# ibm-granite/dolomite-engine

Hardware: NVIDIA H100
Metric: tokens_per_sec (higher is better)
Workload: dtype bf16

## Files before the change

dolomite_engine_b200/csrc/gemm.cu:

```cuda
#include <string.h>

#include "common.cuh"
#include "wgmma.cuh"
#include "../../include/dolomite_b200.h"

using namespace dolo;

namespace {

constexpr int BM = 128;
constexpr int BN = 128;
constexpr int BK = 64;
constexpr int A_STAGE_BYTES = BM * BK * 2;
constexpr int GEMM_THREADS = 384;

constexpr int EPI_SLAB_BYTES = 64 * 128;
constexpr int EPI_BYTES = 2  * 2  * EPI_SLAB_BYTES;
constexpr int EPI_BIAS_BYTES = 2  * 256 * 2;

template <int TN>
struct Ring {
    static_assert(TN == 128 || TN == 256, "tile width 128 or 256");
    static constexpr int STAGES = TN == 256 ? 4 : 6;
    static constexpr int B_BYTES = TN * BK * 2;
// ... 429 lines not shown
            const uint32_t sb = smem_u32(smem_b + stage * B_STAGE_BYTES);
#pragma unroll
            for (int k = 0; k < 4; ++k) {
                const uint64_t adesc = A_MN ? gmma_desc(sa + cw * (BK * 128) + k * 2048, BK * 128, 1024, 1)
                                            : gmma_desc(sa + cw * (64 * 128) + k * 32, 16, 1024, 1);
                const uint64_t bdesc = B_MN ? gmma_desc(sb + k * 2048, BK * 128, 1024, 1)
                                            : gmma_desc(sb + k * 32, 16, 1024, 1);
                Op::template mma<TN>(acc, adesc, bdesc, ((!Op::SPLIT && kb != ti.kb0) || k != 0) ? 1u : 0u);
            }
            wgmma_commit();
            if (kb == min(ti.kb0 + 2, ti.kb1 - 1) && has_c && epi.leader) epi.load_c_prefetch(&maps.c[ti.q], chunk_cols, col0, row0, dgrp);
            if constexpr (Op::SPLIT) {
                wgmma_wait<0>();
                reg_fence<TN / 2>(acc);
                if (lane == 0) mbar_arrive(&empty_bar[stage]);
                if (kb == ti.kb0) {
#pragma unroll
                    for (int i = 0; i < TN / 2; ++i) tot[i] = acc[i];
                } else {
#pragma unroll
                    for (int i = 0; i < TN / 2; ++i) tot[i] += acc[i];
                }
            } else {
                wgmma_wait<1>();
                if (prev_stage >= 0 && lane == 0) mbar_arrive(&empty_bar[prev_stage]);
                prev_stage = stage;
            }
            if (++stage == STAGES) { stage = 0; phase ^= 1; }
        }
        if constexpr (!Op::SPLIT) {
            wgmma_wait<0>();
            reg_fence<TN / 2>(acc);
            if (prev_stage >= 0 && lane == 0) mbar_arrive(&empty_bar[prev_stage]);
        }
        const float(&res)[TN / 2] = Op::SPLIT ? tot : acc;
        float s = 1.f;
        if constexpr (Op::SCALED) s = __ldg(p.a_scale_inv[ti.q]) * __ldg(p.b_scale_inv[ti.q]);
        if (has_bias && wt < TN / 2) epi.bias[wt] = bias_v;
        epi.begin_tile();

        if (p.d_is_f32)
            epi.store<TN, true, Op::SCALED>(res, &maps.d[ti.q], &maps.c[ti.q], col0, row0, dgrp, s, pr.alpha, pr.beta,
                                            has_bias, has_c, Op::GROUPED && p.grouped == 3);
        else
            epi.store<TN, false, Op::SCALED>(res, &maps.d[ti.q], &maps.c[ti.q], col0, row0, dgrp, s, pr.alpha, pr.beta,
                                             has_bias, has_c, false);
    }
    if (epi.leader) tma_store_wait_all<0>();
}

template <bool A_MN, bool B_MN, int TN>
__global__ void __launch_bounds__(GEMM_THREADS, 1)
    gemm_bf16_kernel(const __grid_constant__ GemmMaps maps, const __grid_constant__ GemmParams p) {
    gemm_body<Bf16Ops<A_MN, B_MN>, TN>(maps, p);
}

template <int FA, int FB, bool SPLIT>
__global__ void __launch_bounds__(GEMM_THREADS, 1)
    gemm_fp8_kernel(const __grid_constant__ GemmMaps maps, const __grid_constant__ GemmParams p) {
    gemm_body<Fp8Ops<FA, FB, SPLIT>, 128>(maps, p);
}

int gemm_workers() {
    const int sms = dolo_num_sms() - dolo_option_gemm_sm_margin();
    return sms < 1 ? 1 : sms;
}

template <int TN, void (*KERNEL)(GemmMaps, GemmParams)>
int launch_gemm(const GemmMaps& maps, const GemmParams& p, cudaStream_t st) {
    constexpr int smem_bytes = Ring<TN>::SMEM_BYTES;
    static bool attr_set = false;
    if (!attr_set) {
        DOLO_CUDA_OK(cudaFuncSetAttribute(KERNEL, cudaFuncAttributeMaxDynamicSharedMemorySize, smem_bytes));
        attr_set = true;
    }
    const int sms = gemm_workers();
    const int grid = p.num_tiles < sms ? p.num_tiles : sms;
    KERNEL<<<grid, GEMM_THREADS, smem_bytes, st>>>(maps, p);
    DOLO_LAUNCH_OK("gemm");
    return DOLO_OK;
}

int choose_tile_n(int n, const int64_t* M, const int64_t* N) {
    const int forced = dolo_option_gemm_tile_n();
    if (forced != 0) return forced;
    const int64_t w = gemm_workers();
    int64_t t128 = 0, t256 = 0;
    for (int q = 0; q < n; ++q) {
        const int64_t mb = (M[q] + BM - 1) / BM;
        t128 += mb * ((N[q] + 127) / 128);
        t256 += mb * ((N[q] + 255) / 256);
    }
    const double c128 = double((t128 + w - 1) / w);
    const double c256 = double((t256 + w - 1) / w) * TILE256_COST;
    return c256 < c128 ? 256 : 128;
}

}

struct GroupArgs {
    int mode = 0;
    const int* a_row_index = nullptr;
    int64_t a_rows = 0;
    const int* m_tile_group = nullptr;
    int64_t b_group_rows = 0;
    const int* group_k_offsets = nullptr;
    int num_groups = 1;
    int64_t d_group_stride = 0;
    int64_t b_total_outer = 0;
    int64_t bias_group_stride = 0;
};

struct GemmProblemArgs {
    const void* A; int64_t lda;
    const void* B; int64_t ldb;
    void* D; int64_t ldd;
    const void* C; int64_t ldc;
    const void* bias;
    float alpha, beta;
    int64_t M, N, K;
    const float* a_scale_inv = nullptr;
    const float* b_scale_inv = nullptr;
};

static int setup_problem(GemmMaps& maps, GemmParams& p, int q, const GemmProblemArgs& g, int ab, int a_mn_major,
                         int b_mn_major, int d_is_f32, const GroupArgs& ga, int tile_n) {
    const int64_t M = g.M, N = g.N, K = g.K;
    if (ab == 1) {
        DOLO_REQUIRE(M > 0 && N > 0 && K > 0, "gemm_fp8: empty problem (M=%lld N=%lld K=%lld)", (long long)M,
                     (long long)N, (long long)K);
        DOLO_REQUIRE(K % 16 == 0 && N % 16 == 0, "gemm_fp8: K=%lld and N=%lld must be multiples of 16", (long long)K,
                     (long long)N);
        DOLO_REQUIRE(g.lda % 16 == 0 && g.ldb % 16 == 0 && g.lda >= K && g.ldb >= K,
                     "gemm_fp8: lda / ldb must be >= K and multiples of 16 (16-byte aligned fp8 rows)");
        DOLO_REQUIRE(g.a_scale_inv != nullptr && g.b_scale_inv != nullptr, "gemm_fp8: missing scale_inv pointer");
        p.a_scale_inv[q] = g.a_scale_inv;
        p.b_scale_inv[q] = g.b_scale_inv;
    }
    DOLO_REQUIRE(K > 0, "gemm: K must be > 0");
    DOLO_REQUIRE(g.lda * ab % 16 == 0 && g.ldb * ab % 16 == 0 && g.ldd % (d_is_f32 ? 4 : 8) == 0,
                 "gemm: leading dimensions must keep 16-byte alignment");
    {
        const int64_t per = d_is_f32 ? 4 : 8;
        DOLO_REQUIRE(g.ldd >= (N + per - 1) / per * per,
                     "gemm: ldd=%lld must cover N=%lld rounded up to 16 bytes (the TMA store writes that segment)",
                     (long long)g.ldd, (long long)N);
    }
    DOLO_REQUIRE(g.C == nullptr || g.ldc % (d_is_f32 ? 4 : 8) == 0, "gemm: ldc alignment");
    DOLO_REQUIRE((reinterpret_cast<uintptr_t>(g.bias) & 3) == 0, "gemm: bias must be 4-byte aligned");
    DOLO_REQUIRE(M < (1ll << 31) && N < (1ll << 31) && K < (1ll << 31), "gemm: dimension too large");
// ... 30 lines not shown
        rc = dolo_make_tmap(&maps.b[q], g.B, ab, 3, dims3, strides3, box3, DOLO_SW_128);
    } else {
        dims[0] = uint64_t(N); dims[1] = uint64_t(K); strides[1] = uint64_t(g.ldb) * 2;
        box[0] = 64; box[1] = BK;
        rc = dolo_make_tmap(&maps.b[q], g.B, ab, 2, dims, strides, box, DOLO_SW_128);
    }
    if (rc) return rc;
    {
        const uint64_t eb = d_is_f32 ? 4 : 2;
        const int64_t groups = ga.mode == 2 ? ga.num_groups : 1;
        const int64_t group_stride = ga.mode == 2 ? ga.d_group_stride : M * g.ldd;
        uint64_t ddims[3] = {uint64_t(N), uint64_t(M), uint64_t(groups)};
        uint64_t dstrides[3] = {eb, uint64_t(g.ldd) * eb, uint64_t(group_stride) * eb};
        const uint32_t dbox[3] = {uint32_t(128 / eb), 64, 1};
        rc = dolo_make_tmap(&maps.d[q], g.D, int(eb), 3, ddims, dstrides, dbox, DOLO_SW_128);
        if (rc) return rc;
        if (g.C != nullptr) {
            dstrides[1] = uint64_t(g.ldc) * eb;
            if (ga.mode != 2) dstrides[2] = uint64_t(M * g.ldc) * eb;
            rc = dolo_make_tmap(&maps.c[q], g.C, int(eb), 3, ddims, dstrides, dbox, DOLO_SW_128);
            if (rc) return rc;
        }
    }
    Problem& pr = p.pr[q];
    pr.D = g.D;
    pr.C = g.C;
    pr.bias = static_cast<const __nv_bfloat16*>(g.bias);
    pr.ldd = g.ldd;
    pr.ldc = g.ldc;
    pr.M = int(M);
    pr.N = int(N);
    pr.alpha = g.alpha;
    pr.beta = g.C ? g.beta : 0.f;
    pr.hint_a = pr.hint_b = TMA_HINT_NORMAL;
    if (ab == 2 && dolo_option_gemm_l2_hints() && ga.mode == 0 && K >= 4096 && (M + N) * K * 2 > (24ll << 20)) {
        const bool a_smaller = M <= N;
        pr.hint_a = a_smaller ? TMA_HINT_EVICT_LAST : TMA_HINT_EVICT_FIRST;
        pr.hint_b = a_smaller ? TMA_HINT_EVICT_FIRST : TMA_HINT_EVICT_LAST;
    }
    pr.num_m = int((M + BM - 1) / BM);
    pr.num_n = int((N + tile_n - 1) / tile_n);
    pr.num_kb = int((K * ab + 127) / 128);
    {
        const int64_t panel_bytes = int64_t(BM) * K * ab;
        int64_t gm = (12ll << 20) / (panel_bytes > 0 ? panel_bytes : 1);
        if (gm < 4) gm = 4;
        if (gm > 64) gm = 64;
        pr.group_m = int(gm);
    }
    return DOLO_OK;
}

template <int TN>
static int dispatch_layout(int a_mn_major, int b_mn_major, const GemmMaps& maps, const GemmParams& p, cudaStream_t st) {
    if (!a_mn_major && !b_mn_major) return launch_gemm<TN, gemm_bf16_kernel<false, false, TN>>(maps, p, st);
    if (!a_mn_major && b_mn_major) return launch_gemm<TN, gemm_bf16_kernel<false, true, TN>>(maps, p, st);
    if (a_mn_major && !b_mn_major) return launch_gemm<TN, gemm_bf16_kernel<true, false, TN>>(maps, p, st);
    return launch_gemm<TN, gemm_bf16_kernel<true, true, TN>>(maps, p, st);
}

static int dispatch(int tile_n, int a_mn_major, int b_mn_major, const GemmMaps& maps, const GemmParams& p, cudaStream_t st) {
    return tile_n == 256 ? dispatch_layout<256>(a_mn_major, b_mn_major, maps, p, st)
                         : dispatch_layout<128>(a_mn_major, b_mn_major, maps, p, st);
}

template <int FA, int FB>
static int dispatch_fp8_split(int split, const GemmMaps& maps, const GemmParams& p, cudaStream_t st) {
    return split ? launch_gemm<BN, gemm_fp8_kernel<FA, FB, true>>(maps, p, st)
                 : launch_gemm<BN, gemm_fp8_kernel<FA, FB, false>>(maps, p, st);
}

static int dispatch_fp8(int a_fmt, int b_fmt, int split, const GemmMaps& maps, const GemmParams& p, cudaStream_t st) {
    if (a_fmt == 0 && b_fmt == 0) return dispatch_fp8_split<0, 0>(split, maps, p, st);
    if (a_fmt == 0 && b_fmt == 1) return dispatch_fp8_split<0, 1>(split, maps, p, st);
    if (a_fmt == 1 && b_fmt == 0) return dispatch_fp8_split<1, 0>(split, maps, p, st);
    return dispatch_fp8_split<1, 1>(split, maps, p, st);
}

static int gemm_impl(const void* A, int64_t lda, int a_mn_major, const void* B, int64_t ldb, int b_mn_major, void* D,
                     int64_t ldd, int d_is_f32, const void* C, int64_t ldc, float alpha, float beta, const void* bias,
                     int64_t M, int64_t N, int64_t K, int flags, void* stream, const GroupArgs& ga) {
    DOLO_REQUIRE(M >= 0 && N >= 0 && K >= 0, "gemm: negative dimension");
    if (M == 0 || N == 0) return DOLO_OK;
    const bool tma_store = (flags & DOLO_GEMM_FLAG_TMA_STORE) != 0;
    DOLO_REQUIRE(!tma_store || (!d_is_f32 && C == nullptr), "gemm: TMA-store epilogue needs bf16 D and no C");
    const int tile_n = ga.mode == 0 ? choose_tile_n(1, &M, &N) : BN;
    GemmMaps maps;
    GemmParams p;
    memset(&p, 0, sizeof(p));
    GemmProblemArgs g{A, lda, B, ldb, D, ldd, C, ldc, bias, alpha, beta, M, N, K};
    int rc = setup_problem(maps, p, 0, g, 2, a_mn_major, b_mn_major, d_is_f32, ga, tile_n);
    if (rc) return rc;
    p.n_prob = 1;
    p.pr[0].tile_start = 0;
    p.num_tiles = p.pr[0].num_m * p.pr[0].num_n * (ga.mode >= 2 ? ga.num_groups : 1);
    p.d_is_f32 = d_is_f32;
    p.grouped = ga.mode;
    p.m_tile_group = ga.m_tile_group;
    p.a_row_index = ga.a_row_index;
    p.b_group_rows = int(ga.b_group_rows);
    p.group_k_offsets = ga.group_k_offsets;
    p.num_groups = ga.num_groups;
    p.bias_group_stride = ga.bias_group_stride;
    return dispatch(tile_n, a_mn_major, b_mn_major, maps, p, static_cast<cudaStream_t>(stream));
}

extern "C" int dolomite_b200_gemm_bf16_wgrad_multi(int n_problems, const void* const* dY, const int64_t* ld_dy,
                                                   const void* const* X, const int64_t* ld_x, float* const* dW,
                                                   const int64_t* ld_dw, const int64_t* M, const int64_t* N, int64_t K,
                                                   const float* alpha, const int* accumulate, void* stream) {
    DOLO_REQUIRE(n_problems >= 1 && n_problems <= MAXP, "wgrad_multi: between 1 and %d problems per launch", MAXP);
    for (int q = 0; q < n_problems; ++q) DOLO_REQUIRE(M[q] > 0 && N[q] > 0, "wgrad_multi: empty problem %d", q);
    const int tile_n = choose_tile_n(n_problems, M, N);
    GemmMaps maps;
    GemmParams p;
    memset(&p, 0, sizeof(p));
    int tiles = 0;
    for (int q = 0; q < n_problems; ++q) {
        GemmProblemArgs g{dY[q], ld_dy[q], X[q], ld_x[q], dW[q], ld_dw[q], accumulate[q] ? dW[q] : nullptr, ld_dw[q], nullptr,
                          alpha[q], 1.f, M[q], N[q], K};
        int rc = setup_problem(maps, p, q, g, 2, 1, 1, 1, GroupArgs(), tile_n);
        if (rc) return rc;
        p.pr[q].tile_start = tiles;
        tiles += p.pr[q].num_m * p.pr[q].num_n;
    }
    p.n_prob = n_problems;
    p.num_tiles = tiles;
    p.d_is_f32 = 1;
    p.grouped = 0;
    p.num_groups = 1;
    return dispatch(tile_n, 1, 1, maps, p, static_cast<cudaStream_t>(stream));
}

extern "C" int dolomite_b200_gemm_bf16_tile_n(int n_problems, const int64_t* M, const int64_t* N, int* tile_n,
                                              float* cost_256_over_128) {
    DOLO_REQUIRE(n_problems >= 1 && n_problems <= MAXP && M != nullptr && N != nullptr && tile_n != nullptr,
                 "gemm_bf16_tile_n: between 1 and %d problems, non-null M, N and tile_n", MAXP);
    *tile_n = choose_tile_n(n_problems, M, N);
    if (cost_256_over_128 != nullptr) *cost_256_over_128 = float(TILE256_COST);
    return DOLO_OK;
}

extern "C" int dolomite_b200_gemm_bf16(const void* A, int64_t lda, int a_mn_major, const void* B, int64_t ldb,
                                       int b_mn_major, void* D, int64_t ldd, int d_is_f32, const void* C, int64_t ldc,
                                       float alpha, float beta, const void* bias, int64_t M, int64_t N, int64_t K,
                                       int flags, void* stream) {
    if (flags & DOLO_GEMM_FLAG_SPLITK_ACCUMULATE) {
        DOLO_REQUIRE(d_is_f32 && bias == nullptr && (C == nullptr || (C == D && beta == 1.f)),
                     "gemm: split-K accumulate needs fp32 D, no bias and C == D with beta == 1");
        const int64_t tiles = ((M + BM - 1) / BM) * ((N + BN - 1) / BN);
        const int64_t num_kb = (K + BK - 1) / BK;
        const int sms = dolo_num_sms();
        int best_s = 1;
        double best = 1e30;
        for (int s = 1; s <= 16; ++s) {
            if (s > 1 && num_kb / s < 8) break;
            const double waves = double((tiles * s + sms - 1) / sms) / double(s);
            if (waves < best - 1e-9) { best = waves; best_s = s; }
        }
        GroupArgs ga;
        ga.mode = 3;
        ga.num_groups = best_s;
        return gemm_impl(A, lda, a_mn_major, B, ldb, b_mn_major, D, ldd, 1, nullptr, 0, alpha, 0.f, nullptr, M, N, K, 0,
                         stream, ga);
    }
    return gemm_impl(A, lda, a_mn_major, B, ldb, b_mn_major, D, ldd, d_is_f32, C, ldc, alpha, beta, bias, M, N, K, flags,
                     stream, GroupArgs());
}

static int grouped_m_impl(const void* A, int64_t lda, int64_t a_rows, const int32_t* a_row_index, const void* B,
                          int64_t ldb, int b_mn_major, void* D, int64_t ldd, const void* bias, int64_t ld_bias,
                          float alpha, int64_t M_max, int64_t N, int64_t K, const int32_t* m_tile_group, int num_groups,
                          int flags, void* stream) {
    DOLO_REQUIRE(M_max % BM == 0, "grouped gemm: M_max=%lld must be a multiple of %d (padded expert segments)",
                 (long long)M_max, BM);
    DOLO_REQUIRE(!b_mn_major || K % 8 == 0, "grouped gemm: MN-major B needs K %% 8 == 0 (K=%lld)", (long long)K);
    DOLO_REQUIRE(m_tile_group != nullptr && num_groups > 0, "grouped gemm: missing group table");
    if (a_row_index != nullptr) {
        DOLO_REQUIRE(!b_mn_major && a_rows > 0, "grouped gemm (gather): K-major B and a_rows > 0 needed");
        DOLO_REQUIRE((reinterpret_cast<uintptr_t>(a_row_index) & 15) == 0,
                     "grouped gemm (gather): row index must be 16-byte aligned");
    }
    DOLO_REQUIRE(bias == nullptr || (ld_bias >= N && ld_bias % 2 == 0),
                 "grouped gemm: ld_bias=%lld must be even and >= N=%lld", (long long)ld_bias, (long long)N);
    GroupArgs ga;
    ga.mode = 1;
    ga.a_row_index = a_row_index;
    ga.a_rows = a_rows;
    ga.m_tile_group = m_tile_group;
    ga.num_groups = num_groups;
    ga.b_group_rows = N;
    ga.b_total_outer = N * num_groups;
    ga.bias_group_stride = bias != nullptr ? ld_bias : 0;
    return gemm_impl(A, lda, 0, B, ldb, b_mn_major, D, ldd, 0, nullptr, 0, alpha, 0.f, bias, M_max, N, K, flags, stream,
                     ga);
}

extern "C" int dolomite_b200_gemm_bf16_grouped_m(const void* A, int64_t lda, const void* B, int64_t ldb, int b_mn_major,
                                                 void* D, int64_t ldd, float alpha, int64_t M_max, int64_t N, int64_t K,
                                                 const int32_t* m_tile_group, int num_groups, int flags, void* stream) {
    return grouped_m_impl(A, lda, 0, nullptr, B, ldb, b_mn_major, D, ldd, nullptr, 0, alpha, M_max, N, K, m_tile_group,
                          num_groups, flags, stream);
}

extern "C" int dolomite_b200_gemm_bf16_grouped_m_gather(const void* A, int64_t lda, int64_t a_rows,
                                                        const int32_t* a_row_index, const void* B, int64_t ldb, void* D,
                                                        int64_t ldd, float alpha, int64_t M_max, int64_t N, int64_t K,
                                                        const int32_t* m_tile_group, int num_groups, int flags,
                                                        void* stream) {
    DOLO_REQUIRE(a_row_index != nullptr, "grouped gemm (gather): missing row index");
    return grouped_m_impl(A, lda, a_rows, a_row_index, B, ldb, 0, D, ldd, nullptr, 0, alpha, M_max, N, K, m_tile_group,
                          num_groups, flags, stream);
}

extern "C" int dolomite_b200_gemm_bf16_grouped_m_bias(const void* A, int64_t lda, int64_t a_rows,
                                                      const int32_t* a_row_index, const void* B, int64_t ldb,
                                                      int b_mn_major, void* D, int64_t ldd, const void* bias,
                                                      int64_t ld_bias, float alpha, int64_t M_max, int64_t N, int64_t K,
                                                      const int32_t* m_tile_group, int num_groups, int flags,
                                                      void* stream) {
// ... 67 lines not shown
```

dolomite_engine_b200/_lib.py:

```python

from __future__ import annotations

import ctypes
import os
from ctypes import c_char_p, c_float, c_int, c_int64, c_uint32, c_void_p

_HERE = os.path.dirname(os.path.abspath(__file__))
LIB_PATH = os.path.join(_HERE, "lib", "libdolomite_b200.so")


class DolomiteB200Error(RuntimeError):
    pass


_P = c_void_p
_I = c_int
_L = c_int64
_F = c_float
_U = c_uint32

SIGNATURES: dict[str, tuple] = {
    "dolomite_b200_last_error": (c_char_p, []),
    "dolomite_b200_abi_version": (_I, []),
    "dolomite_b200_device_info": (_I, [_P, _P, _P]),
    "dolomite_b200_set_option": (_I, [c_char_p, _I]),
    "dolomite_b200_get_option": (_I, [c_char_p, _P]),
    "dolomite_b200_rmsnorm_fwd": (_I, [_P, _P, _P, _P, _L, _I, _F, _P]),
    "dolomite_b200_rmsnorm_bwd_workspace_bytes": (_L, [_I]),
    "dolomite_b200_rmsnorm_bwd": (_I, [_P, _P, _P, _P, _P, _P, _P, _P, _L, _I, _P]),
    "dolomite_b200_rope_qk_inplace": (_I, [_P, _L, _L, _I, _I, _I, _P, _P, _P, _I, _L, _I, _P]),
    "dolomite_b200_layernorm_fwd": (_I, [_P, _P, _P, _P, _P, _P, _L, _I, _F, _P]),
    "dolomite_b200_layernorm_bwd_workspace_bytes": (_L, [_I]),
    "dolomite_b200_layernorm_bwd": (_I, [_P, _P, _P, _P, _P, _P, _P, _P, _P, _P, _L, _I, _P]),
    "dolomite_b200_act_fwd": (_I, [_I, _I, _P, _P, _L, _L, _P]),
    "dolomite_b200_act_bwd": (_I, [_I, _I, _P, _P, _P, _P, _L, _L, _P]),
    "dolomite_b200_act_bwd_segmented": (_I, [_I, _I, _P, _P, _P, _P, _L, _L, _P, _I, _P]),
    "dolomite_b200_gelu_fwd": (_I, [_P, _P, _L, _P]),
    "dolomite_b200_gelu_bwd": (_I, [_P, _P, _P, _P, _L, _L, _P]),
    "dolomite_b200_swiglu_fwd": (_I, [_P, _P, _L, _L, _P]),
    "dolomite_b200_swiglu_bwd": (_I, [_P, _P, _P, _L, _L, _P]),
    "dolomite_b200_swiglu_bwd_bias": (_I, [_P, _P, _P, _P, _L, _L, _P]),
    "dolomite_b200_embedding_fwd": (_I, [_P, _P, _P, _L, _I, _L, _F, _P]),
    "dolomite_b200_embedding_bwd": (_I, [_P, _P, _P, _L, _I, _L, _F, _P]),
    "dolomite_b200_embedding_fwd_neft": (_I, [_P, _P, _P, _L, _I, _L, _U, _U, _F, _P]),
    "dolomite_b200_cross_entropy_fwd_bwd": (_I, [_P, _L, _P, _P, _P, _P, _P, _L, _L, _L, _F, _F, _P]),
    "dolomite_b200_cross_entropy_count": (_I, [_P, _L, _L, _P, _P]),
    "dolomite_b200_cross_entropy_rows": (_I, [_P, _L, _P, _P, _P, _P, _L, _L, _L, _F, _F, _P]),
    "dolomite_b200_cross_entropy_mean": (_I, [_P, _L, _P, _P, _P]),
    "dolomite_b200_colsum_accum": (_I, [_P, _L, _P, _L, _L, _F, _P]),
    "dolomite_b200_colsum_accum_segmented": (_I, [_P, _L, _P, _L, _L, _P, _I, _F, _P]),
    "dolomite_b200_scale_bf16_by_device_scalar": (_I, [_P, _L, _P, _P]),
    "dolomite_b200_add_scaled": (_I, [_P, _P, _P, _F, _L, _P]),
    "dolomite_b200_dropout_fwd": (_I, [_P, _P, _P, _L, _F, _F, _U, _U, _P]),
    "dolomite_b200_dropout_bwd": (_I, [_P, _P, _L, _F, _F, _U, _U, _P]),
    "dolomite_b200_sumsq_workspace_bytes": (_L, []),
    "dolomite_b200_sumsq_accum": (_I, [_P, _L, _P, _P, _P]),
    "dolomite_b200_clip_coef": (_I, [_P, _F, _P, _P, _P]),
    "dolomite_b200_adamw_step": (_I, [_P, _P, _P, _P, _P, _L, _F, _F, _F, _F, _F, _L, _P, _P]),
    "dolomite_b200_cast_f32_to_bf16": (_I, [_P, _P, _L, _P]),
    "dolomite_b200_accum_bf16_into_f32": (_I, [_P, _P, _F, _L, _P]),
    "dolomite_b200_gemm_bf16": (
        _I,
        [_P, _L, _I, _P, _L, _I, _P, _L, _I, _P, _L, _F, _F, _P, _L, _L, _L, _I, _P],
    ),
    "dolomite_b200_gemm_bf16_wgrad_multi": (_I, [_I, _P, _P, _P, _P, _P, _P, _P, _P, _L, _P, _P, _P]),
    "dolomite_b200_gemm_bf16_tile_n": (_I, [_I, _P, _P, _P, _P]),
    "dolomite_b200_gemm_fp8": (
        _I,
        [_P, _L, _I, _P, _L, _I, _P, _P, _P, _L, _I, _P, _L, _F, _F, _P, _L, _L, _L, _I, _P],
    ),
    "dolomite_b200_gemm_fp8_wgrad_multi": (
        _I,
        [_I, _P, _P, _P, _P, _P, _P, _P, _P, _P, _P, _L, _P, _P, _I, _I, _I, _P],
    ),
    "dolomite_b200_fp8_cast": (_I, [_P, _L, _L, _L, _I, _P, _P, _P, _P, _P]),
    "dolomite_b200_fp8_scaling_update": (_I, [_P, _I, _L, _P, _P, _F, _P]),
    "dolomite_b200_gemm_bf16_grouped_m": (_I, [_P, _L, _P, _L, _I, _P, _L, _F, _L, _L, _L, _P, _I, _I, _P]),
    "dolomite_b200_gemm_bf16_grouped_k": (_I, [_P, _L, _P, _L, _P, _L, _F, _F, _L, _L, _L, _P, _I, _P]),
    "dolomite_b200_moe_max_rows": (_L, [_L, _I, _I]),
    "dolomite_b200_moe_route": (_I, [_P, _L, _I, _I, _P, _P, _P, _P, _P, _P, _P, _P, _P, _P]),
    "dolomite_b200_gemm_bf16_grouped_m_gather": (_I, [_P, _L, _L, _P, _P, _L, _P, _L, _F, _L, _L, _L, _P, _I, _I, _P]),
    "dolomite_b200_gemm_bf16_grouped_m_bias": (
        _I,
        [_P, _L, _L, _P, _P, _L, _I, _P, _L, _P, _L, _F, _L, _L, _L, _P, _I, _I, _P],
    ),
    "dolomite_b200_moe_gather": (_I, [_P, _P, _P, _P, _L, _I, _I, _I, _P]),
    "dolomite_b200_moe_combine": (_I, [_P, _P, _P, _P, _P, _L, _I, _I, _F, _P]),
    "dolomite_b200_moe_combine_bwd": (_I, [_P, _P, _P, _P, _P, _P, _P, _L, _I, _I, _I, _F, _P]),
    "dolomite_b200_moe_token_sum": (_I, [_P, _P, _P, _L, _I, _I, _P]),
    "dolomite_b200_moe_router_bwd": (_I, [_P, _P, _P, _P, _L, _I, _I, _P]),
    "dolomite_b200_moe_aux_partial_floats": (_L, [_L, _I]),
    "dolomite_b200_moe_aux_stats": (_I, [_P, _P, _L, _L, _I, _I, _P, _P, _P]),
    "dolomite_b200_moe_aux_finalize": (_I, [_P, _I, _L, _F, _P, _P, _P, _P]),
    "dolomite_b200_moe_router_bwd_aux": (_I, [_P, _P, _P, _P, _P, _P, _P, _L, _L, _I, _I, _P]),
    "dolomite_b200_attn_varlen_fwd": (_I, [_P, _L, _P, _P, _P, _I, _L, _I, _I, _I, _I, _F, _P]),
    "dolomite_b200_attn_decode": (_I, [_P, _L, _P, _P, _P, _P, _I, _L, _I, _I, _I, _F, _P]),
    "dolomite_b200_attn_varlen_bwd_workspace_bytes": (_L, [_L, _I, _I, _I]),
    "dolomite_b200_attn_varlen_bwd": (
        _I,
        [_P, _P, _L, _P, _P, _P, _P, _I, _L, _I, _I, _I, _I, _F, _P, _P],
    ),
    "dolomite_b200_attn_varlen_fwd_dropout": (_I, [_P, _L, _P, _P, _P, _I, _L, _I, _I, _I, _I, _F, _F, _U, _U, _P]),
    "dolomite_b200_attn_varlen_bwd_dropout": (
        _I,
        [_P, _P, _L, _P, _P, _P, _P, _I, _L, _I, _I, _I, _I, _F, _F, _U, _U, _P, _P],
    ),
    "dolomite_b200_attn_varlen_fwd_alibi": (_I, [_P, _L, _P, _P, _P, _I, _L, _I, _I, _I, _I, _F, _F, _U, _U, _P, _P]),
    "dolomite_b200_attn_varlen_bwd_alibi": (
        _I,
        [_P, _P, _L, _P, _P, _P, _P, _I, _L, _I, _I, _I, _I, _F, _F, _U, _U, _P, _P, _P],
    ),
    "dolomite_b200_attn_decode_alibi": (_I, [_P, _L, _P, _P, _P, _P, _I, _L, _I, _I, _I, _F, _P, _P]),
    "dolomite_b200_attn_cache": (_I, [_P, _L, _P, _P, _P, _P, _P, _I, _I, _I, _L, _I, _I, _I, _F, _P]),
    "dolomite_b200_attn_cache_alibi": (_I, [_P, _L, _P, _P, _P, _P, _P, _I, _I, _I, _L, _I, _I, _I, _F, _P, _P]),
}

_lib = None


def lib_available() -> bool:
    return os.path.exists(LIB_PATH)


def load():
    global _lib
    if _lib is not None:
        return _lib
    if not os.path.exists(LIB_PATH):
        raise DolomiteB200Error(
            f"{LIB_PATH} not found. Build it with `python -m dolomite_engine_b200.build` "
            "(or __graft_entry__.build()); there is no CPU / PyTorch fallback for the hot path."
        )
    lib = ctypes.CDLL(LIB_PATH)
    for name, (res, args) in SIGNATURES.items():
        fn = getattr(lib, name)
        fn.restype = res
        fn.argtypes = args
    _lib = lib
    for item in filter(None, os.environ.get("DOLO_OPTIONS", "").split(",")):
        key, _, value = item.partition("=")
        if lib.dolomite_b200_set_option(key.strip().encode(), int(value)) != 0:
            raise DolomiteB200Error(f"DOLO_OPTIONS: {lib.dolomite_b200_last_error().decode()}")
    return lib


def check(rc: int, what: str = "") -> None:
    if rc != 0:
        msg = load().dolomite_b200_last_error()
        raise DolomiteB200Error(f"{what}: rc={rc}: {msg.decode() if msg else '?'}")


KERNELS_PER_CALL = {
    "dolomite_b200_rmsnorm_fwd": 1, "dolomite_b200_rmsnorm_bwd": 2, "dolomite_b200_rope_qk_inplace": 1,
    "dolomite_b200_layernorm_fwd": 1, "dolomite_b200_layernorm_bwd": 3, "dolomite_b200_gelu_fwd": 1,
    "dolomite_b200_gelu_bwd": 1, "dolomite_b200_swiglu_fwd": 1, "dolomite_b200_swiglu_bwd": 1, "dolomite_b200_swiglu_bwd_bias": 1,
    "dolomite_b200_act_fwd": 1, "dolomite_b200_act_bwd": 1,
    "dolomite_b200_embedding_fwd": 1, "dolomite_b200_embedding_fwd_neft": 1,
    "dolomite_b200_embedding_bwd": 1, "dolomite_b200_cross_entropy_fwd_bwd": 3, "dolomite_b200_colsum_accum": 1,
    "dolomite_b200_scale_bf16_by_device_scalar": 1, "dolomite_b200_add_scaled": 1, "dolomite_b200_sumsq_accum": 2,
    "dolomite_b200_clip_coef": 1, "dolomite_b200_adamw_step": 1, "dolomite_b200_cast_f32_to_bf16": 1,
    "dolomite_b200_accum_bf16_into_f32": 1, "dolomite_b200_gemm_bf16": 1, "dolomite_b200_attn_varlen_fwd": 1,
    "dolomite_b200_attn_varlen_bwd": 3, "dolomite_b200_attn_varlen_fwd_dropout": 1, "dolomite_b200_attn_varlen_bwd_dropout": 3,
    "dolomite_b200_attn_varlen_fwd_alibi": 1, "dolomite_b200_attn_varlen_bwd_alibi": 3, "dolomite_b200_attn_decode_alibi": 1,
    "dolomite_b200_dropout_fwd": 1, "dolomite_b200_dropout_bwd": 1, "dolomite_b200_gemm_bf16_tile_n": 0,
    "dolomite_b200_moe_aux_stats": 2,
}
launch_counts: dict[str, int] = {}


def reset_launch_counts() -> None:
    launch_counts.clear()


def total_kernel_launches() -> int:
    return sum(KERNELS_PER_CALL.get(k, 1) * v for k, v in launch_counts.items())


def call(name: str, *args):
    lib = load()
    launch_counts[name] = launch_counts.get(name, 0) + 1
    rc = getattr(lib, name)(*args)
    if rc != 0:
        msg = lib.dolomite_b200_last_error()
        raise DolomiteB200Error(f"{name} failed (rc={rc}): {msg.decode() if msg else '?'}")
```

dolomite_engine_b200/kernels.py:

```python

from __future__ import annotations

import torch

from . import _lib

_BF16 = torch.bfloat16


def set_option(key: str, value: int) -> None:
    _lib.call("dolomite_b200_set_option", key.encode(), int(value))


def get_option(key: str) -> int:
    import ctypes

    v = ctypes.c_int(0)
    _lib.call("dolomite_b200_get_option", key.encode(), ctypes.addressof(v))
    return int(v.value)


def _stream() -> int:
    return torch.cuda.current_stream().cuda_stream

# ... 431 lines not shown
        if d_is_f32 or c is not None:
            flags &= ~GEMM_TMA_STORE
        if d_is_f32 and c is out and beta == 1.0 and bias is None and wgrad_splitk:
            flags |= GEMM_SPLITK_ACCUMULATE
    if gemm_timer is not None:
        e0, e1 = torch.cuda.Event(enable_timing=True), torch.cuda.Event(enable_timing=True)
        e0.record()
    _lib.call(
        "dolomite_b200_gemm_bf16", a.data_ptr(), a.stride(0), int(a_mn), b.data_ptr(), b.stride(0), int(b_mn),
        out.data_ptr(), out.stride(0), d_is_f32, _ptr(c), 0 if c is None else c.stride(0), alpha, beta, _ptr(bias),
        M, N, K, flags, _stream(),
    )
    if gemm_timer is not None:
        e1.record()
        gemm_timer.append((2.0 * M * N * K, e0, e1))
    return out


def gemm_wgrad_multi(problems: list[tuple], n_rows: int | None = None) -> None:
    import ctypes

    n = len(problems)
    assert 1 <= n <= 4
    K = problems[0][0].shape[0] if n_rows is None else n_rows
    P, L, F, I = ctypes.c_void_p * n, ctypes.c_int64 * n, ctypes.c_float * n, ctypes.c_int * n
    for dy, x, dw, _, _ in problems:
        _req(dy, _BF16, "dy"), _req(x, _BF16, "x"), _req(dw, torch.float32, "dw")
        assert dy.shape[0] == K and x.shape[0] == K and dy.stride(1) == 1 and x.stride(1) == 1 and dw.stride(1) == 1
        assert dw.shape == (dy.shape[1], x.shape[1])
    if gemm_timer is not None:
        e0, e1 = torch.cuda.Event(enable_timing=True), torch.cuda.Event(enable_timing=True)
        e0.record()
    _lib.call(
        "dolomite_b200_gemm_bf16_wgrad_multi", n, P(*[q[0].data_ptr() for q in problems]), L(*[q[0].stride(0) for q in problems]),
        P(*[q[1].data_ptr() for q in problems]), L(*[q[1].stride(0) for q in problems]), P(*[q[2].data_ptr() for q in problems]),
        L(*[q[2].stride(0) for q in problems]), L(*[q[0].shape[1] for q in problems]), L(*[q[1].shape[1] for q in problems]),
        K, F(*[float(q[3]) for q in problems]), I(*[int(bool(q[4])) for q in problems]), _stream(),
    )
    if gemm_timer is not None:
        e1.record()
        gemm_timer.append((sum(2.0 * K * q[0].shape[1] * q[1].shape[1] for q in problems), e0, e1))


def gemm_tile_n(shapes: list[tuple[int, int]]) -> tuple[int, float]:
    import ctypes

    n = len(shapes)
    tile_n, cost = ctypes.c_int(0), ctypes.c_float(0.0)
    _lib.call("dolomite_b200_gemm_bf16_tile_n", n, (ctypes.c_int64 * n)(*[s[0] for s in shapes]),
              (ctypes.c_int64 * n)(*[s[1] for s in shapes]), ctypes.addressof(tile_n), ctypes.addressof(cost))
    return int(tile_n.value), float(cost.value)


E4M3, E5M2 = 0, 1
FP8_MAX = {E4M3: 448.0, E5M2: 57344.0}
_U8 = torch.uint8


def fp8_cast(x, fmt: int, scale, *, plain: bool = True, transpose: bool = False, amax=None, out=None, out_t=None):
    _req(x, _BF16, "x"), _req(scale, torch.float32, "scale")
    assert x.dim() == 2 and x.stride(1) == 1 and (plain or transpose)
    rows, cols = x.shape
    if plain and out is None:
        out = torch.empty(rows, cols, dtype=_U8, device=x.device)
    if transpose and out_t is None:
        out_t = torch.empty(cols, rows, dtype=_U8, device=x.device)
    if amax is not None:
        _req(amax, torch.float32, "amax")
    _lib.call("dolomite_b200_fp8_cast", x.data_ptr(), x.stride(0), rows, cols, fmt, scale.data_ptr(),
              _ptr(out) if plain else None, _ptr(out_t) if transpose else None, _ptr(amax), _stream())
    return (out if plain else None), (out_t if transpose else None)


def fp8_scaling_update(amax_history, scale, scale_inv, fmt: int) -> None:
    _req(amax_history, torch.float32, "amax_history"), _req(scale, torch.float32, "scale")
    _req(scale_inv, torch.float32, "scale_inv")
    L, n = amax_history.shape
    assert amax_history.is_contiguous() and scale.numel() == n and scale_inv.numel() == n
    _lib.call("dolomite_b200_fp8_scaling_update", amax_history.data_ptr(), L, n, scale.data_ptr(), scale_inv.data_ptr(),
              FP8_MAX[fmt], _stream())


def gemm_fp8(a, a_fmt: int, a_scale_inv, b, b_fmt: int, b_scale_inv, *, out=None, out_dtype=_BF16, c=None, alpha=1.0,
             beta=0.0, bias=None, split_accumulate: bool = False):
    _req(a, _U8, "a"), _req(b, _U8, "b"), _req(a_scale_inv, torch.float32, "a_scale_inv")
    _req(b_scale_inv, torch.float32, "b_scale_inv")
    assert a.dim() == 2 and b.dim() == 2 and a.stride(1) == 1 and b.stride(1) == 1
    M, K = a.shape
    N, Kb = b.shape
    if K != Kb:
        raise _lib.DolomiteB200Error(f"gemm_fp8: contraction mismatch {K} vs {Kb}")
    if out is None:
        out = torch.empty(M, N, dtype=out_dtype, device=a.device)
    assert out.stride(1) == 1 and out.shape == (M, N)
    if c is not None:
        assert c.dtype == out.dtype and c.stride(1) == 1
    if gemm_timer is not None:
        e0, e1 = torch.cuda.Event(enable_timing=True), torch.cuda.Event(enable_timing=True)
        e0.record()
    _lib.call(
        "dolomite_b200_gemm_fp8", a.data_ptr(), a.stride(0), a_fmt, b.data_ptr(), b.stride(0), b_fmt, a_scale_inv.data_ptr(),
        b_scale_inv.data_ptr(), out.data_ptr(), out.stride(0), int(out.dtype == torch.float32), _ptr(c),
        0 if c is None else c.stride(0), alpha, beta, _ptr(bias), M, N, K, int(split_accumulate), _stream(),
    )
    if gemm_timer is not None:
        e1.record()
# ... 349 lines not shown
```

include/dolomite_b200.h:

```cpp
#ifndef DOLOMITE_B200_H
#define DOLOMITE_B200_H

#include <stdint.h>

#ifdef __cplusplus
extern "C" {
#endif

#define DOLOMITE_B200_ABI_VERSION 1

#define DOLO_OK 0
#define DOLO_ERR_INVALID (-1)
#define DOLO_ERR_CUDA (-2)

const char* dolomite_b200_last_error(void);
int dolomite_b200_abi_version(void);
int dolomite_b200_device_info(int* sm_count, int* cc_major, int* cc_minor);
int dolomite_b200_set_option(const char* key, int value);
int dolomite_b200_get_option(const char* key, int* value);

int dolomite_b200_rmsnorm_fwd(const void* x, const void* w, void* y, float* rstd, int64_t T, int H, float eps,
                              void* stream);
int64_t dolomite_b200_rmsnorm_bwd_workspace_bytes(int H);
int dolomite_b200_rmsnorm_bwd(const void* dy, const void* x, const void* w, const float* rstd, const void* dx_add,
// ... 75 lines not shown
int dolomite_b200_colsum_accum_segmented(const void* x, int64_t ldx, float* out, int64_t ld_out, int64_t N,
                                         const int32_t* seg_offsets, int num_segments, float scale, void* stream);
int dolomite_b200_scale_bf16_by_device_scalar(void* x, int64_t n, const float* scale, void* stream);

int dolomite_b200_add_scaled(const void* a, const void* b, void* out, float alpha, int64_t n, void* stream);

int dolomite_b200_dropout_fwd(const void* x, const void* residual, void* out, int64_t n, float p, float post_mul,
                              uint32_t key0, uint32_t key1, void* stream);
int dolomite_b200_dropout_bwd(const void* dy, void* dx, int64_t n, float p, float pre_mul, uint32_t key0, uint32_t key1,
                              void* stream);

int64_t dolomite_b200_sumsq_workspace_bytes(void);
int dolomite_b200_sumsq_accum(const float* g, int64_t n, float* out, void* workspace, void* stream);
int dolomite_b200_clip_coef(const float* sumsq, float max_norm, float* coef_out, float* norm_out, void* stream);
int dolomite_b200_adamw_step(float* p, const float* g, float* m, float* v, void* p_bf16, int64_t n, float lr,
                             float beta1, float beta2, float eps, float weight_decay, int64_t step,
                             const float* clip_coef, void* stream);
int dolomite_b200_cast_f32_to_bf16(const float* src, void* dst, int64_t n, void* stream);
int dolomite_b200_accum_bf16_into_f32(const void* src, float* dst, float scale, int64_t n, void* stream);

int dolomite_b200_attn_decode(const void* qkv, int64_t row_stride, const void* k_cache, const void* v_cache, const int32_t* lens,
                              void* out, int batch, int64_t L_max, int n_groups, int q_per_group, int head_dim,
                              float softmax_scale, void* stream);
int dolomite_b200_attn_decode_alibi(const void* qkv, int64_t row_stride, const void* k_cache, const void* v_cache,
                                    const int32_t* lens, void* out, int batch, int64_t L_max, int n_groups, int q_per_group,
                                    int head_dim, float softmax_scale, const float* alibi_slopes, void* stream);

int dolomite_b200_attn_cache(const void* qkv, int64_t row_stride, const int32_t* cu_new, const int32_t* past,
                             const void* k_cache, const void* v_cache, void* out, int batch, int max_new, int max_end,
                             int64_t L_max, int n_groups, int q_per_group, int head_dim, float softmax_scale, void* stream);
int dolomite_b200_attn_cache_alibi(const void* qkv, int64_t row_stride, const int32_t* cu_new, const int32_t* past,
                                   const void* k_cache, const void* v_cache, void* out, int batch, int max_new, int max_end,
                                   int64_t L_max, int n_groups, int q_per_group, int head_dim, float softmax_scale,
                                   const float* alibi_slopes, void* stream);

#define DOLO_GEMM_FLAG_TMA_STORE 1
#define DOLO_GEMM_FLAG_SPLITK_ACCUMULATE 2
#define DOLO_GEMM_FLAG_CTA_PAIR 4
#define DOLO_GEMM_FLAG_NO_CTA_PAIR 8
#define DOLO_GEMM_FLAG_DIRECT_EPILOGUE 16
#define DOLO_GEMM_FLAG_F32_TMA_EPILOGUE 32
int dolomite_b200_gemm_bf16(const void* A, int64_t lda, int a_mn_major, const void* B, int64_t ldb, int b_mn_major,
                            void* D, int64_t ldd, int d_is_f32, const void* C, int64_t ldc, float alpha, float beta,
                            const void* bias, int64_t M, int64_t N, int64_t K, int flags, void* stream);

int dolomite_b200_gemm_bf16_wgrad_multi(int n_problems, const void* const* dY, const int64_t* ld_dy, const void* const* X,
                                        const int64_t* ld_x, float* const* dW, const int64_t* ld_dw, const int64_t* M,
                                        const int64_t* N, int64_t K, const float* alpha, const int* accumulate,
                                        void* stream);

int dolomite_b200_gemm_bf16_tile_n(int n_problems, const int64_t* M, const int64_t* N, int* tile_n,
                                   float* cost_256_over_128);

int dolomite_b200_gemm_fp8(const void* A, int64_t lda, int a_fmt, const void* B, int64_t ldb, int b_fmt,
                           const float* a_scale_inv, const float* b_scale_inv, void* D, int64_t ldd, int d_is_f32,
                           const void* C, int64_t ldc, float alpha, float beta, const void* bias, int64_t M, int64_t N,
                           int64_t K, int split_accumulate, void* stream);
int dolomite_b200_gemm_fp8_wgrad_multi(int n_problems, const void* const* dYt, const int64_t* ld_dyt, const void* const* Xt,
                                       const int64_t* ld_xt, const float* const* dy_scale_inv,
                                       const float* const* x_scale_inv, float* const* dW, const int64_t* ld_dw,
                                       const int64_t* M, const int64_t* N, int64_t K, const float* alpha,
                                       const int* accumulate, int dy_fmt, int x_fmt, int split_accumulate, void* stream);
int dolomite_b200_fp8_cast(const void* x, int64_t ldx, int64_t rows, int64_t cols, int fmt, const float* scale, void* out,
                           void* out_t, float* amax, void* stream);
int dolomite_b200_fp8_scaling_update(float* amax_history, int history_len, int64_t n_slots, float* scale, float* scale_inv,
                                     float fp8_max, void* stream);

int dolomite_b200_gemm_bf16_grouped_m(const void* A, int64_t lda, const void* B, int64_t ldb, int b_mn_major, void* D,
                                      int64_t ldd, float alpha, int64_t M_max, int64_t N, int64_t K,
                                      const int32_t* m_tile_group, int num_groups, int flags, void* stream);
int dolomite_b200_gemm_bf16_grouped_m_gather(const void* A, int64_t lda, int64_t a_rows, const int32_t* a_row_index,
                                             const void* B, int64_t ldb, void* D, int64_t ldd, float alpha, int64_t M_max,
                                             int64_t N, int64_t K, const int32_t* m_tile_group, int num_groups, int flags,
                                             void* stream);
int dolomite_b200_gemm_bf16_grouped_m_bias(const void* A, int64_t lda, int64_t a_rows, const int32_t* a_row_index,
                                           const void* B, int64_t ldb, int b_mn_major, void* D, int64_t ldd,
                                           const void* bias, int64_t ld_bias, float alpha, int64_t M_max, int64_t N,
                                           int64_t K, const int32_t* m_tile_group, int num_groups, int flags,
                                           void* stream);
int dolomite_b200_gemm_bf16_grouped_k(const void* A, int64_t lda, const void* B, int64_t ldb, float* D, int64_t ldd,
                                      float alpha, float beta, int64_t M, int64_t N, int64_t K_max,
                                      const int32_t* group_k_offsets, int num_groups, void* stream);

int64_t dolomite_b200_moe_max_rows(int64_t T, int E, int k);
int dolomite_b200_moe_route(const void* router_logits, int64_t T, int E, int k, int32_t* sel_idx, float* sel_w,
                            int32_t* counts, int32_t* offsets_padded, int32_t* m_tile_group, int32_t* cursors,
                            int32_t* row_of_slot, int32_t* slot_of_row, int32_t* token_of_row, void* stream);
int dolomite_b200_moe_gather(const void* x, void* xg, const int32_t* slot_of_row, const int32_t* offsets_padded,
                             int64_t T, int E, int k, int H, void* stream);
int dolomite_b200_moe_combine(const void* yg, const int32_t* row_of_slot, const float* sel_w, const void* c, void* out,
                              int64_t T, int k, int H, float alpha, void* stream);
int dolomite_b200_moe_combine_bwd(const void* dy, const void* yg, const int32_t* slot_of_row,
                                  const int32_t* offsets_padded, const float* sel_w, void* dyg, float* dw, int64_t T,
                                  int E, int k, int H, float alpha, void* stream);
int dolomite_b200_moe_token_sum(const void* dxg, const int32_t* row_of_slot, void* dx, int64_t T, int k, int H,
                                void* stream);
int dolomite_b200_moe_router_bwd(const int32_t* sel_idx, const float* sel_w, const float* dw, void* dlogits, int64_t T,
                                 int E, int k, void* stream);

int64_t dolomite_b200_moe_aux_partial_floats(int64_t T_real, int E);
int dolomite_b200_moe_aux_stats(const void* router_logits, const int32_t* sel_idx, int64_t T, int64_t T_real, int E, int k,
                                float* partial, float* acc, void* stream);
int dolomite_b200_moe_aux_finalize(const float* acc, int E, int64_t n_tokens, float coef, float* aux, float* c,
                                   float* loss, void* stream);
int dolomite_b200_moe_router_bwd_aux(const void* router_logits, const int32_t* sel_idx, const float* sel_w,
                                     const float* dw, const float* c, const float* s, void* dlogits, int64_t T,
// ... 34 lines not shown
```

Before: 18090.

## Split dense GEMM columns into 256-wide and 128-wide tile launches to balance waves

Adds a cost model that, for K >= 1024 with no forced tile width, looks for a column split point where the left part uses 256-wide tiles and the remainder uses 128-wide tiles. When the modeled wave cost beats the best single-width choice by a margin, the GEMM is issued as two launches over offset B/D/C/bias pointers. This aims to reduce wave quantization and tail waste, at the cost of an extra kernel launch and reliance on a crude cost constant.

New measurement: 18330 (median of 6 runs). +1.3%, better.

```diff
diff --git a/dolomite_engine_b200/csrc/gemm.cu b/dolomite_engine_b200/csrc/gemm.cu
--- a/dolomite_engine_b200/csrc/gemm.cu
+++ b/dolomite_engine_b200/csrc/gemm.cu
@@ -549,6 +549,21 @@
     return c256 < c128 ? 256 : 128;
 }
 
+int64_t split_cols(int64_t M, int64_t N, int64_t K) {
+    if (dolo_option_gemm_tile_n() != 0 || K < 1024) return 0;
+    const int64_t w = gemm_workers();
+    const int64_t mb = (M + BM - 1) / BM, nb = (N + 255) / 256;
+    auto waves = [w](int64_t tiles) { return double((tiles + w - 1) / w); };
+    const double c128 = waves(mb * ((N + 127) / 128)), c256 = waves(mb * nb) * TILE256_COST;
+    double best = (c256 < c128 ? c256 : c128) - 0.5;
+    int64_t n1 = 0;
+    for (int64_t j = 1; j < nb; ++j) {
+        const double c = waves(mb * j) * TILE256_COST + waves(mb * ((N - 256 * j + 127) / 128));
+        if (c < best) { best = c; n1 = 256 * j; }
+    }
+    return n1;
+}
+
 }
 
 struct GroupArgs {
@@ -712,12 +727,13 @@
 
 static int gemm_impl(const void* A, int64_t lda, int a_mn_major, const void* B, int64_t ldb, int b_mn_major, void* D,
                      int64_t ldd, int d_is_f32, const void* C, int64_t ldc, float alpha, float beta, const void* bias,
-                     int64_t M, int64_t N, int64_t K, int flags, void* stream, const GroupArgs& ga) {
+                     int64_t M, int64_t N, int64_t K, int flags, void* stream, const GroupArgs& ga, int tile_n = 0) {
     DOLO_REQUIRE(M >= 0 && N >= 0 && K >= 0, "gemm: negative dimension");
     if (M == 0 || N == 0) return DOLO_OK;
     const bool tma_store = (flags & DOLO_GEMM_FLAG_TMA_STORE) != 0;
     DOLO_REQUIRE(!tma_store || (!d_is_f32 && C == nullptr), "gemm: TMA-store epilogue needs bf16 D and no C");
-    const int tile_n = ga.mode == 0 ? choose_tile_n(1, &M, &N) : BN;
+    if (ga.mode != 0) tile_n = BN;
+    else if (tile_n == 0) tile_n = choose_tile_n(1, &M, &N);
     GemmMaps maps;
     GemmParams p;
     memset(&p, 0, sizeof(p));
@@ -796,6 +812,22 @@
         ga.num_groups = best_s;
         return gemm_impl(A, lda, a_mn_major, B, ldb, b_mn_major, D, ldd, 1, nullptr, 0, alpha, 0.f, nullptr, M, N, K, 0,
                          stream, ga);
+    }
+    const int64_t n1 = split_cols(M, N, K);
+    if (n1 > 0) {
+        const int64_t eb = d_is_f32 ? 4 : 2, per = 16 / eb;
+        DOLO_REQUIRE(ldd >= (N + per - 1) / per * per,
+                     "gemm: ldd=%lld must cover N=%lld rounded up to 16 bytes (the TMA store writes that segment)",
+                     (long long)ldd, (long long)N);
+        const char* B2 = static_cast<const char*>(B) + (b_mn_major ? n1 : n1 * ldb) * 2;
+        char* D2 = static_cast<char*>(D) + n1 * eb;
+        const char* C2 = C == nullptr ? nullptr : static_cast<const char*>(C) + n1 * eb;
+        const char* bias2 = bias == nullptr ? nullptr : static_cast<const char*>(bias) + n1 * 2;
+        int rc = gemm_impl(A, lda, a_mn_major, B, ldb, b_mn_major, D, ldd, d_is_f32, C, ldc, alpha, beta, bias, M, n1, K,
+                           flags, stream, GroupArgs(), 256);
+        if (rc) return rc;
+        return gemm_impl(A, lda, a_mn_major, B2, ldb, b_mn_major, D2, ldd, d_is_f32, C2, ldc, alpha, beta, bias2, M, N - n1,
+                         K, flags, stream, GroupArgs(), 128);
     }
     return gemm_impl(A, lda, a_mn_major, B, ldb, b_mn_major, D, ldd, d_is_f32, C, ldc, alpha, beta, bias, M, N, K, flags,
                      stream, GroupArgs());
```

## Split dense GEMM along M into 256-wide and 128-wide launches with PDL overlap

Applied to the files above, without the earlier changes.

A planner splits dense bf16 GEMMs along M. The leading rows run with 256-wide N tiles sized to fill whole waves of workers, and the remainder runs with 128-wide tiles. The second launch uses programmatic dependent launch: the kernel signals dependents at entry and waits at exit, so the tail launch can start while the first is still draining. The aim is to cut wave-quantization waste, at the cost of an extra launch and a cost model based on a fixed 256-vs-128 tile cost ratio.

Result: faster. 18440 before, 18640 after (median of 6 runs) (+1.1%).

```diff
diff --git a/dolomite_engine_b200/_lib.py b/dolomite_engine_b200/_lib.py
--- a/dolomite_engine_b200/_lib.py
+++ b/dolomite_engine_b200/_lib.py
@@ -65,6 +65,7 @@
     ),
     "dolomite_b200_gemm_bf16_wgrad_multi": (_I, [_I, _P, _P, _P, _P, _P, _P, _P, _P, _L, _P, _P, _P]),
     "dolomite_b200_gemm_bf16_tile_n": (_I, [_I, _P, _P, _P, _P]),
+    "dolomite_b200_gemm_bf16_plan": (_I, [_L, _L, _P, _P]),
     "dolomite_b200_gemm_fp8": (
         _I,
         [_P, _L, _I, _P, _L, _I, _P, _P, _P, _L, _I, _P, _L, _F, _F, _P, _L, _L, _L, _I, _P],
@@ -163,6 +164,7 @@
     "dolomite_b200_attn_varlen_bwd": 3, "dolomite_b200_attn_varlen_fwd_dropout": 1, "dolomite_b200_attn_varlen_bwd_dropout": 3,
     "dolomite_b200_attn_varlen_fwd_alibi": 1, "dolomite_b200_attn_varlen_bwd_alibi": 3, "dolomite_b200_attn_decode_alibi": 1,
     "dolomite_b200_dropout_fwd": 1, "dolomite_b200_dropout_bwd": 1, "dolomite_b200_gemm_bf16_tile_n": 0,
+    "dolomite_b200_gemm_bf16_plan": 0,
     "dolomite_b200_moe_aux_stats": 2,
 }
 launch_counts: dict[str, int] = {}
diff --git a/dolomite_engine_b200/csrc/gemm.cu b/dolomite_engine_b200/csrc/gemm.cu
--- a/dolomite_engine_b200/csrc/gemm.cu
+++ b/dolomite_engine_b200/csrc/gemm.cu
@@ -505,7 +505,9 @@
 template <bool A_MN, bool B_MN, int TN>
 __global__ void __launch_bounds__(GEMM_THREADS, 1)
     gemm_bf16_kernel(const __grid_constant__ GemmMaps maps, const __grid_constant__ GemmParams p) {
+    asm volatile("griddepcontrol.launch_dependents;" ::: "memory");
     gemm_body<Bf16Ops<A_MN, B_MN>, TN>(maps, p);
+    asm volatile("griddepcontrol.wait;" ::: "memory");
 }
 
 template <int FA, int FB, bool SPLIT>
@@ -520,7 +522,7 @@
 }
 
 template <int TN, void (*KERNEL)(GemmMaps, GemmParams)>
-int launch_gemm(const GemmMaps& maps, const GemmParams& p, cudaStream_t st) {
+int launch_gemm(const GemmMaps& maps, const GemmParams& p, cudaStream_t st, bool follow_on = false) {
     constexpr int smem_bytes = Ring<TN>::SMEM_BYTES;
     static bool attr_set = false;
     if (!attr_set) {
@@ -529,7 +531,21 @@
     }
     const int sms = gemm_workers();
     const int grid = p.num_tiles < sms ? p.num_tiles : sms;
-    KERNEL<<<grid, GEMM_THREADS, smem_bytes, st>>>(maps, p);
+    if (!follow_on) {
+        KERNEL<<<grid, GEMM_THREADS, smem_bytes, st>>>(maps, p);
+    } else {
+        cudaLaunchConfig_t cfg = {};
+        cfg.gridDim = dim3(unsigned(grid));
+        cfg.blockDim = dim3(GEMM_THREADS);
+        cfg.dynamicSmemBytes = smem_bytes;
+        cfg.stream = st;
+        cudaLaunchAttribute attr[1];
+        attr[0].id = cudaLaunchAttributeProgrammaticStreamSerialization;
+        attr[0].val.programmaticStreamSerializationAllowed = 1;
+        cfg.attrs = attr;
+        cfg.numAttrs = 1;
+        DOLO_CUDA_OK(cudaLaunchKernelEx(&cfg, KERNEL, maps, p));
+    }
     DOLO_LAUNCH_OK("gemm");
     return DOLO_OK;
 }
@@ -547,6 +563,23 @@
     const double c128 = double((t128 + w - 1) / w);
     const double c256 = double((t256 + w - 1) / w) * TILE256_COST;
     return c256 < c128 ? 256 : 128;
+}
+
+struct GemmPlan {
+    int tile_n;
+    int64_t split_m;
+};
+
+GemmPlan plan_dense(int64_t M, int64_t N) {
+    const int tile_n = choose_tile_n(1, &M, &N);
+    if (dolo_option_gemm_tile_n() != 0) return {tile_n, 0};
+    const int64_t w = gemm_workers();
+    const int64_t mb = (M + BM - 1) / BM, n128 = (N + 127) / 128, n256 = (N + 255) / 256;
+    const int64_t m1 = (mb * n256 / w) * w / n256;
+    if (m1 == 0 || m1 == mb) return {tile_n, 0};
+    const double unsplit = tile_n == 256 ? double((mb * n256 + w - 1) / w) * TILE256_COST : double((mb * n128 + w - 1) / w);
+    const double split = double((m1 * n256 + w - 1) / w) * TILE256_COST + double(((mb - m1) * n128 + w - 1) / w);
+    return split < unsplit ? GemmPlan{256, m1 * BM} : GemmPlan{tile_n, 0};
 }
 
 }
@@ -685,16 +718,18 @@
 }
 
 template <int TN>
-static int dispatch_layout(int a_mn_major, int b_mn_major, const GemmMaps& maps, const GemmParams& p, cudaStream_t st) {
-    if (!a_mn_major && !b_mn_major) return launch_gemm<TN, gemm_bf16_kernel<false, false, TN>>(maps, p, st);
-    if (!a_mn_major && b_mn_major) return launch_gemm<TN, gemm_bf16_kernel<false, true, TN>>(maps, p, st);
-    if (a_mn_major && !b_mn_major) return launch_gemm<TN, gemm_bf16_kernel<true, false, TN>>(maps, p, st);
-    return launch_gemm<TN, gemm_bf16_kernel<true, true, TN>>(maps, p, st);
-}
-
-static int dispatch(int tile_n, int a_mn_major, int b_mn_major, const GemmMaps& maps, const GemmParams& p, cudaStream_t st) {
-    return tile_n == 256 ? dispatch_layout<256>(a_mn_major, b_mn_major, maps, p, st)
-                         : dispatch_layout<128>(a_mn_major, b_mn_major, maps, p, st);
+static int dispatch_layout(int a_mn_major, int b_mn_major, const GemmMaps& maps, const GemmParams& p, cudaStream_t st,
+                           bool follow_on) {
+    if (!a_mn_major && !b_mn_major) return launch_gemm<TN, gemm_bf16_kernel<false, false, TN>>(maps, p, st, follow_on);
+    if (!a_mn_major && b_mn_major) return launch_gemm<TN, gemm_bf16_kernel<false, true, TN>>(maps, p, st, follow_on);
+    if (a_mn_major && !b_mn_major) return launch_gemm<TN, gemm_bf16_kernel<true, false, TN>>(maps, p, st, follow_on);
+    return launch_gemm<TN, gemm_bf16_kernel<true, true, TN>>(maps, p, st, follow_on);
+}
+
+static int dispatch(int tile_n, int a_mn_major, int b_mn_major, const GemmMaps& maps, const GemmParams& p, cudaStream_t st,
+                    bool follow_on = false) {
+    return tile_n == 256 ? dispatch_layout<256>(a_mn_major, b_mn_major, maps, p, st, follow_on)
+                         : dispatch_layout<128>(a_mn_major, b_mn_major, maps, p, st, follow_on);
 }
 
 template <int FA, int FB>
@@ -710,16 +745,10 @@
     return dispatch_fp8_split<1, 1>(split, maps, p, st);
 }
 
-static int gemm_impl(const void* A, int64_t lda, int a_mn_major, const void* B, int64_t ldb, int b_mn_major, void* D,
-                     int64_t ldd, int d_is_f32, const void* C, int64_t ldc, float alpha, float beta, const void* bias,
-                     int64_t M, int64_t N, int64_t K, int flags, void* stream, const GroupArgs& ga) {
-    DOLO_REQUIRE(M >= 0 && N >= 0 && K >= 0, "gemm: negative dimension");
-    if (M == 0 || N == 0) return DOLO_OK;
-    const bool tma_store = (flags & DOLO_GEMM_FLAG_TMA_STORE) != 0;
-    DOLO_REQUIRE(!tma_store || (!d_is_f32 && C == nullptr), "gemm: TMA-store epilogue needs bf16 D and no C");
-    const int tile_n = ga.mode == 0 ? choose_tile_n(1, &M, &N) : BN;
-    GemmMaps maps;
-    GemmParams p;
+static int setup_launch(GemmMaps& maps, GemmParams& p, const void* A, int64_t lda, int a_mn_major, const void* B,
+                        int64_t ldb, int b_mn_major, void* D, int64_t ldd, int d_is_f32, const void* C, int64_t ldc,
+                        float alpha, float beta, const void* bias, int64_t M, int64_t N, int64_t K, const GroupArgs& ga,
+                        int tile_n) {
     memset(&p, 0, sizeof(p));
     GemmProblemArgs g{A, lda, B, ldb, D, ldd, C, ldc, bias, alpha, beta, M, N, K};
     int rc = setup_problem(maps, p, 0, g, 2, a_mn_major, b_mn_major, d_is_f32, ga, tile_n);
@@ -735,7 +764,55 @@
     p.group_k_offsets = ga.group_k_offsets;
     p.num_groups = ga.num_groups;
     p.bias_group_stride = ga.bias_group_stride;
-    return dispatch(tile_n, a_mn_major, b_mn_major, maps, p, static_cast<cudaStream_t>(stream));
+    return DOLO_OK;
+}
+
+static int check_dims(int64_t M, int64_t N, int64_t K, int d_is_f32, const void* C, int flags) {
+    DOLO_REQUIRE(M >= 0 && N >= 0 && K >= 0, "gemm: negative dimension");
+    const bool tma_store = (flags & DOLO_GEMM_FLAG_TMA_STORE) != 0;
+    DOLO_REQUIRE(!tma_store || (!d_is_f32 && C == nullptr), "gemm: TMA-store epilogue needs bf16 D and no C");
+    return DOLO_OK;
+}
+
+static int gemm_impl(const void* A, int64_t lda, int a_mn_major, const void* B, int64_t ldb, int b_mn_major, void* D,
+                     int64_t ldd, int d_is_f32, const void* C, int64_t ldc, float alpha, float beta, const void* bias,
+                     int64_t M, int64_t N, int64_t K, int flags, void* stream, const GroupArgs& ga) {
+    int rc = check_dims(M, N, K, d_is_f32, C, flags);
+    if (rc || M == 0 || N == 0) return rc;
+    GemmMaps maps;
+    GemmParams p;
+    rc = setup_launch(maps, p, A, lda, a_mn_major, B, ldb, b_mn_major, D, ldd, d_is_f32, C, ldc, alpha, beta, bias, M, N,
+                      K, ga, BN);
+    if (rc) return rc;
+    return dispatch(BN, a_mn_major, b_mn_major, maps, p, static_cast<cudaStream_t>(stream));
+}
+
+static int gemm_dense(const void* A, int64_t lda, int a_mn_major, const void* B, int64_t ldb, int b_mn_major, void* D,
+                      int64_t ldd, int d_is_f32, const void* C, int64_t ldc, float alpha, float beta, const void* bias,
+                      int64_t M, int64_t N, int64_t K, int flags, void* stream) {
+    int rc = check_dims(M, N, K, d_is_f32, C, flags);
+    if (rc || M == 0 || N == 0) return rc;
+    const GemmPlan plan = plan_dense(M, N);
+    const cudaStream_t st = static_cast<cudaStream_t>(stream);
+    GemmMaps maps;
+    GemmParams p;
+    const int64_t m1 = plan.split_m > 0 ? plan.split_m : M;
+    rc = setup_launch(maps, p, A, lda, a_mn_major, B, ldb, b_mn_major, D, ldd, d_is_f32, C, ldc, alpha, beta, bias, m1, N,
+                      K, GroupArgs(), plan.tile_n);
+    if (rc) return rc;
+    if (plan.split_m == 0) return dispatch(plan.tile_n, a_mn_major, b_mn_major, maps, p, st);
+    const int64_t eb = d_is_f32 ? 4 : 2;
+    const char* A2 = static_cast<const char*>(A) + (a_mn_major ? m1 : m1 * lda) * 2;
+    char* D2 = static_cast<char*>(D) + m1 * ldd * eb;
+    const char* C2 = C != nullptr ? static_cast<const char*>(C) + m1 * ldc * eb : nullptr;
+    GemmMaps maps2;
+    GemmParams p2;
+    rc = setup_launch(maps2, p2, A2, lda, a_mn_major, B, ldb, b_mn_major, D2, ldd, d_is_f32, C2, ldc, alpha, beta, bias,
+                      M - m1, N, K, GroupArgs(), 128);
+    if (rc) return rc;
+    rc = dispatch(256, a_mn_major, b_mn_major, maps, p, st);
+    if (rc) return rc;
+    return dispatch(128, a_mn_major, b_mn_major, maps2, p2, st, dolo_option_gemm_sm_margin() == 0);
 }
 
 extern "C" int dolomite_b200_gemm_bf16_wgrad_multi(int n_problems, const void* const* dY, const int64_t* ld_dy,
@@ -774,6 +851,15 @@
     return DOLO_OK;
 }
 
+extern "C" int dolomite_b200_gemm_bf16_plan(int64_t M, int64_t N, int* tile_n, int64_t* split_m) {
+    DOLO_REQUIRE(M > 0 && N > 0 && tile_n != nullptr && split_m != nullptr,
+                 "gemm_bf16_plan: M, N > 0 and non-null tile_n and split_m");
+    const GemmPlan plan = plan_dense(M, N);
+    *tile_n = plan.split_m > 0 ? 0 : plan.tile_n;
+    *split_m = plan.split_m;
+    return DOLO_OK;
+}
+
 extern "C" int dolomite_b200_gemm_bf16(const void* A, int64_t lda, int a_mn_major, const void* B, int64_t ldb,
                                        int b_mn_major, void* D, int64_t ldd, int d_is_f32, const void* C, int64_t ldc,
                                        float alpha, float beta, const void* bias, int64_t M, int64_t N, int64_t K,
@@ -797,8 +883,8 @@
         return gemm_impl(A, lda, a_mn_major, B, ldb, b_mn_major, D, ldd, 1, nullptr, 0, alpha, 0.f, nullptr, M, N, K, 0,
                          stream, ga);
     }
-    return gemm_impl(A, lda, a_mn_major, B, ldb, b_mn_major, D, ldd, d_is_f32, C, ldc, alpha, beta, bias, M, N, K, flags,
-                     stream, GroupArgs());
+    return gemm_dense(A, lda, a_mn_major, B, ldb, b_mn_major, D, ldd, d_is_f32, C, ldc, alpha, beta, bias, M, N, K, flags,
+                      stream);
 }
 
 static int grouped_m_impl(const void* A, int64_t lda, int64_t a_rows, const int32_t* a_row_index, const void* B,
diff --git a/dolomite_engine_b200/kernels.py b/dolomite_engine_b200/kernels.py
--- a/dolomite_engine_b200/kernels.py
+++ b/dolomite_engine_b200/kernels.py
@@ -507,6 +507,14 @@
     return int(tile_n.value), float(cost.value)
 
 
+def gemm_plan(M: int, N: int) -> tuple[int, int]:
+    import ctypes
+
+    tile_n, split_m = ctypes.c_int(0), ctypes.c_int64(0)
+    _lib.call("dolomite_b200_gemm_bf16_plan", M, N, ctypes.addressof(tile_n), ctypes.addressof(split_m))
+    return int(tile_n.value), int(split_m.value)
+
+
 E4M3, E5M2 = 0, 1
 FP8_MAX = {E4M3: 448.0, E5M2: 57344.0}
 _U8 = torch.uint8
diff --git a/include/dolomite_b200.h b/include/dolomite_b200.h
--- a/include/dolomite_b200.h
+++ b/include/dolomite_b200.h
@@ -151,6 +151,8 @@
 int dolomite_b200_gemm_bf16_tile_n(int n_problems, const int64_t* M, const int64_t* N, int* tile_n,
                                    float* cost_256_over_128);
 
+int dolomite_b200_gemm_bf16_plan(int64_t M, int64_t N, int* tile_n, int64_t* split_m);
+
 int dolomite_b200_gemm_fp8(const void* A, int64_t lda, int a_fmt, const void* B, int64_t ldb, int b_fmt,
                            const float* a_scale_inv, const float* b_scale_inv, void* D, int64_t ldd, int d_is_f32,
                            const void* C, int64_t ldc, float alpha, float beta, const void* bias, int64_t M, int64_t N,
```
